# hiroharu-kato/neural_renderer

Measured on AMD Instinct MI355X. Metric: rasterize fwd+bwd Mpixels/sec @256x256 batch=64, higher is better.
Workload: dtype f32

## Files before the change

neural_renderer_amd/csrc/nr_backward_pixel_map.hip:

```cpp
#include "nr_device.h"
#include "nr_band_lines.h"
#include "nr_face_gather.h"
#include "nr_k6_tune.h"

#include <atomic>
#include <mutex>
#include <type_traits>

using namespace nr;

namespace {

constexpr int GRP = 10;
constexpr int NGRP = 6;

struct __attribute__((aligned(16))) LineRec {
    int in_rng;
    int out_rng;
    int base;
    int flags;
    float cross, c0, c1, pad;
    float in_c[4];
    float out_c[4];
};
// ... 350 lines not shown
}

__global__ __launch_bounds__(VIS_CHUNK) void k_compact_visible(const unsigned char *__restrict__ flags,
                                                               const int *__restrict__ chunk_count,
                                                               int *__restrict__ vis_list, int *__restrict__ vis_count,
                                                               int *__restrict__ slot_of, int F, int n_chunks,
                                                               const float *__restrict__ faces,
                                                               unsigned *__restrict__ rng, double *__restrict__ scratch,
                                                               int S, int *__restrict__ band_lines, int n_bands, int W,
                                                               int lds_counters, float *__restrict__ zero_faces,
                                                               int zero_listed)
{
    extern __shared__ int s_band[];
    __shared__ int s_wcnt[VIS_CHUNK / 64];
    __shared__ int s_part[VIS_CHUNK / 64];
    const int b = blockIdx.y, chunk = blockIdx.x, tid = threadIdx.x, lane = tid & 63, wave = tid >> 6;
    if (lds_counters)
        for (int i = tid; i < 2 * n_bands; i += VIS_CHUNK) s_band[i] = 0;
    int part = 0;
    for (int c = tid; c < chunk; c += VIS_CHUNK) part += chunk_count[(size_t)b * n_chunks + c];
#pragma unroll
    for (int o = 32; o > 0; o >>= 1) part += __shfl_xor(part, o, WAVE);
    const int fn = chunk * VIS_CHUNK + tid;
    const bool v = fn < F && flags[(size_t)b * F + fn] != 0;
    const unsigned long long m = __ballot(v);
    if (lane == 0) { s_part[wave] = part; s_wcnt[wave] = __popcll(m); }
    __syncthreads();
    int off = 0, own = 0;
    for (int w = 0; w < VIS_CHUNK / 64; ++w) {
        off += s_part[w];
        if (w < wave) off += s_wcnt[w];
        own += s_wcnt[w];
    }
    if (fn < F) {
        const int before = off + __popcll(m & ((1ull << lane) - 1ull));
        slot_of[(size_t)b * F + fn] = v ? before : -1;
        if (zero_faces && (!v || zero_listed)) zero_face(zero_faces + ((size_t)b * F + fn) * 9);
        if (v)
            emit_visible(b, fn, before, F, S, faces, vis_list, rng, scratch,
                         lds_counters ? s_band : band_lines + (size_t)b * 2 * n_bands, n_bands, W);
    }
    if (lds_counters) {
        __syncthreads();
        for (int i = tid; i < 2 * n_bands; i += VIS_CHUNK) {
            const int c = s_band[i];
            if (c) atomicAdd(band_lines + (size_t)b * 2 * n_bands + i, c);
        }
    }
    if (chunk == n_chunks - 1 && tid == 0) {
        int base = 0;
        for (int w = 0; w < VIS_CHUNK / 64; ++w) base += s_part[w];
        vis_count[b] = base + own;
    }
}

template <int NT>
__device__ __forceinline__ int block_excl_scan(int v, int *s_tmp, int *total)
{
    const int tid = threadIdx.x, lane = tid & 63, wave = tid >> 6;
    int inc = v;
#pragma unroll
    for (int o = 1; o < 64; o <<= 1) {
        const int t = __shfl_up(inc, o, WAVE);
        if (lane >= o) inc += t;
    }
    if (lane == 63) s_tmp[wave] = inc;
    __syncthreads();
    int woff = 0, tot = 0;
    for (int w = 0; w < NT / 64; ++w) {
        const int c = s_tmp[w];
        if (w < wave) woff += c;
        tot += c;
    }
    __syncthreads();
    *total = tot;
    return woff + inc - v;
}

__device__ __forceinline__ double signed_eps(float dist, unsigned eps_hi, unsigned eps_lo)
{
    return __hiloint2double((int)((0.0f < dist) ? eps_hi : (eps_hi ^ 0x80000000u)), (int)eps_lo);
}

__global__ __launch_bounds__(256) void k_line_setup(LineSetupArgs a) { line_setup_body(a, (int)blockIdx.x, (int)blockIdx.y); }

__device__ __forceinline__ void band_prefix(const int *cnt, int n2, int *__restrict__ start_out, int *__restrict__ cursor_out,
                                            int *__restrict__ ok_out, size_t cap)
{
    if (threadIdx.x >= 64) return;
    const int lane = threadIdx.x, per = (n2 + 63) / 64;
    int local = 0;
    for (int i = lane * per; i < min(n2, (lane + 1) * per); ++i) local += cnt[i];
    int inc = local;
#pragma unroll
    for (int o = 1; o < 64; o <<= 1) {
        const int t = __shfl_up(inc, o, WAVE);
        if (lane >= o) inc += t;
    }
    int run = inc - local;
    for (int i = lane * per; i < min(n2, (lane + 1) * per); ++i) {
        start_out[i] = run;
        cursor_out[i] = 0;
        run += cnt[i];
    }
    const int total = __shfl(inc, 63, WAVE);
    if (lane == 0) *ok_out = ((size_t)total <= cap) ? 1 : 0;
}

__global__ __launch_bounds__(256) void k_band_scan(const int *__restrict__ band_lines, int *__restrict__ band_start,
                                                   int *__restrict__ band_cursor, int *__restrict__ lines_ok, int n_bands,
                                                   size_t cap, int force_scan)
{
    const size_t o = (size_t)blockIdx.x * 2 * n_bands;
    band_prefix(band_lines + o, 2 * n_bands, band_start + o, band_cursor + o, lines_ok + blockIdx.x, force_scan ? 0 : cap);
}

__global__ __launch_bounds__(256) void k_band_total(const int *__restrict__ chunk_band, int n_sum, int *__restrict__ band_lines,
                                                    int *__restrict__ band_start, int *__restrict__ lines_ok, int n_bands)
{
    const int b = blockIdx.x, n2 = 2 * n_bands;
    const int *rows = chunk_band + (size_t)b * n_sum * n2;
    for (int i = threadIdx.x; i < n2; i += blockDim.x) {
        int t = 0;
        for (int c = 0; c < n_sum; ++c) t += rows[(size_t)c * n2 + i];
        band_lines[(size_t)b * n2 + i] = t;
        band_start[(size_t)b * n2 + i] = 0;
    }
    if (threadIdx.x == 0) lines_ok[b] = 0;
}

struct FastPx {
    int *fi;
    float *g;
    float *c;
    float *bg;
    unsigned *cov;
    int CW;
    int *span;
};

template <bool RGB, bool ALPHA, int NT>
__device__ __forceinline__ void fast_stage(const FastPx &px, const int32_t *__restrict__ fi_map,
                                           const float *__restrict__ rgb_map, const float *__restrict__ alpha_map,
                                           const float *__restrict__ g_rgb, const float *__restrict__ g_alpha, size_t img,
                                           int axis, int band_lo, int nld, int S, int SP)
{
    const int tid = threadIdx.x;
    auto put = [&](int ld, int d1, int fi, float al, float ga, float r, float g, float bl, float gr, float gg, float gb) {
        const int l = ld * SP + d1;
        px.fi[l] = fi;
        if (RGB) {
            *reinterpret_cast<float4 *>(px.g + 4 * (size_t)l) = make_float4(ga, gr, gg, gb);
            *reinterpret_cast<float4 *>(px.c + 4 * (size_t)l) = make_float4(al, r, g, bl);
            if (px.bg && fi < 0) *reinterpret_cast<float4 *>(px.bg) = make_float4(al, r, g, bl);
        } else {
            px.g[l] = ga;
            px.c[l] = al;
            if (px.bg && fi < 0) px.bg[0] = al;
        }
        if (px.cov && fi >= 0) atomicOr(px.cov + ld * px.CW + (d1 >> 5), 1u << (d1 & 31));
    };
    auto put_quad = [&](size_t g, int ld0, int d10, int ld_step, int d1_step) {
        const int4 vf = *reinterpret_cast<const int4 *>(fi_map + g);
        float4 va = make_float4(0, 0, 0, 0), vg = va;
        if (ALPHA) {
            va = *reinterpret_cast<const float4 *>(alpha_map + g);
            vg = *reinterpret_cast<const float4 *>(g_alpha + g);
// ... 1105 lines not shown
                            __builtin_amdgcn_sched_barrier(0);
                            visit(gC, pC, pf + (float)(2 * SEG), a0, a1);
                            used(gC);
                            visit(gD, pD, pf + (float)(3 * SEG), b0, b1);
                            used(gD);
                            __builtin_amdgcn_sched_barrier(0);
                            gp += 4 * (SEG * NC * 4);
                            pp += 4 * SEG;
                            pf += (float)(4 * SEG);
                        }
                        if (const int rem = steps2 - s) {
                            if (rem == 3) load(2, gC, pC);
                            visit(gA, pA, pf, a0, a1);
                            used(gA);
                            if (rem >= 2) {
                                visit(gB, pB, pf + (float)SEG, b0, b1);
                                used(gB);
                            }
                            if (rem == 3) {
                                visit(gC, pC, pf + (float)(2 * SEG), a0, a1);
                                used(gC);
                            }
                        }
                    }
                    A0 = __builtin_amdgcn_mfma_f64_4x4x4f64((double)a0, 1.0, 0.0, 0, 0, 0);
                    A1 = __builtin_amdgcn_mfma_f64_4x4x4f64((double)a1, 1.0, 0.0, 0, 0, 0);
                    A0 = __builtin_amdgcn_mfma_f64_4x4x4f64((double)b0, 1.0, A0, 0, 0, 0);
                    A1 = __builtin_amdgcn_mfma_f64_4x4x4f64((double)b1, 1.0, A1, 0, 0, 0);
                    A0 = __builtin_amdgcn_mfma_f64_4x4x4f64(A0, 1.0, 0.0, 0, 0, 0);
                    A1 = __builtin_amdgcn_mfma_f64_4x4x4f64(A1, 1.0, 0.0, 0, 0, 0);
                }
                if (act && lane == (row << 2)) acc[src] = make_double2(A0, A1);
            }
            wave_lds_handover();
            if (lane < nw) {
                double2 a = make_double2(0.0, 0.0);
                if (has_b && ((pos >> 2) & (team - 1)) == member) a = acc[lane];
                a.x += (double)f0;
                a.y += (double)f1;
                const bool tneg = !dpos;
                const bool neg0 = EXACT || (((__float_as_uint(qq.y) >> 31) != 0) != tneg);
                const bool neg1 = EXACT || (((__float_as_uint(qq.z) >> 31) != 0) != tneg);
                const double t0 = (flags & 2) ? in0 + (neg0 ? a.x : -a.x) : 0.0;
                const double t1 = (flags & 4) ? in1 + (neg1 ? a.y : -a.y) : 0.0;
                const int tgt = hh.w, lpos = tgt & 0x0fffffff;
                double *dst = scratch + ((size_t)b * F + lpos) * 6 + (1 - axis);
                if (t0 != 0.0) atomicAdd(dst + 2 * ((tgt >> 28) & 3), t0);
                if (t1 != 0.0) atomicAdd(dst + 2 * ((tgt >> 30) & 3), t1);
            }
            wave_lds_handover();
        }
    }
}

template <bool RGB, bool ALPHA, int MODE, bool CHUNKED>
__global__ __launch_bounds__(rowk::NT, MODE == K6_FAST ? 5 : 4) void k_bpm_row(
    const int32_t *__restrict__ fi_map, const float *__restrict__ rgb_map, const float *__restrict__ alpha_map,
    const float *__restrict__ g_rgb, const float *__restrict__ g_alpha, double *__restrict__ scratch,
    const int *__restrict__ band_lines, const int *__restrict__ band_start, const int *__restrict__ lines_ok,
    const BandLine *__restrict__ line_buf, size_t cap, int F, int S, int W, int CH, float eps_f, double eps_d, int B,
    uint4 *__restrict__ zero16, size_t n_zero16)
{
    bpm_row_body<RGB, ALPHA, MODE, CHUNKED, false>(fi_map, rgb_map, alpha_map, g_rgb, g_alpha, scratch, band_lines, band_start, lines_ok,
                                                   line_buf, cap, F, S, W, CH, eps_f, eps_d, B, zero16, n_zero16, nullptr, 1u);
}

struct BandRowArgs {
    const int32_t *fi_map;
    const float *rgb_map, *alpha_map, *g_rgb, *g_alpha;
    double *scratch;
    const int *band_lines, *band_start, *lines_ok;
    const BandLine *line_buf;
    size_t cap;
    int F, S, W, B;
    float eps_f;
    double eps_d;
    uint4 *zero16;
    size_t n_zero16;
    const int *zero_slot;
    unsigned zero_epf;
};

template <bool RGB, bool ALPHA, bool DEPTH>
__global__ __launch_bounds__(rowk::NT, 5) void k_band_gather(BandRowArgs r, FaceGatherArgs g, unsigned band_grid, unsigned gather_x)
{
    if (blockIdx.x < band_grid) {
        bpm_row_body<RGB, ALPHA, K6_FAST, false, true>(r.fi_map, r.rgb_map, r.alpha_map, r.g_rgb, r.g_alpha, r.scratch, r.band_lines,
                                                       r.band_start, r.lines_ok, r.line_buf, r.cap, r.F, r.S, r.W, r.S, r.eps_f, r.eps_d,
                                                       r.B, r.zero16, r.n_zero16, r.zero_slot, r.zero_epf);
    } else {
        const unsigned id = blockIdx.x - band_grid;
        face_gather_body<true, DEPTH, false>(g, (int)(id % gather_x), (int)(id / gather_x));
    }
}

__global__ __launch_bounds__(256) void k_bpm_finalize(const double *__restrict__ scratch, const int *__restrict__ slot_of,
                                                      float *__restrict__ grad_faces, int F, int n_faces_total, int add)
{
    const int i = blockIdx.x * blockDim.x + threadIdx.x;
    if (i >= n_faces_total) return;
    const int pos = slot_of[i];
    float *o = grad_faces + (size_t)i * 9;
    if (add) {
        if (pos < 0) return;
        const double *src = scratch + ((size_t)(i / F) * F + pos) * 6;
#pragma unroll
        for (int v = 0; v < 3; v++) {
            o[3 * v + 0] = (float)src[2 * v + 0] + o[3 * v + 0];
            o[3 * v + 1] = (float)src[2 * v + 1] + o[3 * v + 1];
        }
        return;
    }
    double a[6] = {0.0, 0.0, 0.0, 0.0, 0.0, 0.0};
    if (pos >= 0) {
        const double *src = scratch + ((size_t)(i / F) * F + pos) * 6;
#pragma unroll
        for (int k = 0; k < 6; k++) a[k] = src[k];
    }
#pragma unroll
    for (int v = 0; v < 3; v++) {
        o[3 * v + 0] = (float)a[2 * v + 0];
        o[3 * v + 1] = (float)a[2 * v + 1];
        o[3 * v + 2] = 0.0f;
    }
}


struct BpmLayout {
    size_t flags_off, scratch_off, count_off, chunk_off, cband_off, list_off, rng_off, slot_off, band_off, start_off, cursor_off, ok_off,
        lines_off, total, cap;
    int n_chunks;
};

size_t line_capacity(int F, int S)
{
    const size_t want = (size_t)8 * F + (size_t)32 * S + (size_t)(1.2 * (double)S * sqrt((double)F));
    return (want + 2047 - 1088) / 2048 * 2048 + 1088;
}

BpmLayout bpm_layout(int B, int F, int S)
{
    BpmLayout L;
    const size_t n = (size_t)B * F;
    L.flags_off = 0;
    L.scratch_off = align_up(n, 256);
    L.count_off = align_up(L.scratch_off + n * 6 * sizeof(double), 256);
    L.n_chunks = (F + VIS_CHUNK - 1) / VIS_CHUNK;
    L.chunk_off = L.count_off + align_up((size_t)B * sizeof(int), 256);
    L.cband_off = L.chunk_off + align_up((size_t)B * L.n_chunks * sizeof(int), 256);
    L.list_off = L.cband_off + (L.n_chunks <= SMALL_CHUNKS ? align_up((size_t)B * L.n_chunks * 2 * S * sizeof(int), 256) : 0);
    L.rng_off = L.list_off + align_up(n * sizeof(int), 256);
    L.slot_off = L.rng_off + align_up(n * 6 * sizeof(unsigned), 256);
    const size_t per_band = align_up((size_t)B * 2 * S * sizeof(int), 256);
    L.band_off = L.slot_off + align_up(n * sizeof(int), 256);
    L.start_off = L.band_off + per_band;
    L.cursor_off = L.start_off + per_band;
    L.ok_off = L.cursor_off + per_band;
    L.lines_off = L.ok_off + align_up((size_t)B * sizeof(int), 256);
    L.cap = line_capacity(F, S);
    L.total = L.lines_off + (size_t)B * L.cap * sizeof(BandLine);
    return L;
}

struct ListsLayout {
    size_t count_off, list_off, total;
};
ListsLayout lists_layout(int B, int F)
{
    ListsLayout L;
    L.count_off = 0;
    L.list_off = align_up((size_t)B * sizeof(int), 256);
    L.total = L.list_off + (size_t)B * F * sizeof(int);
    return L;
}

// ... 63 lines not shown
    return (rgb && alpha) ? by_mode(T(), T()) : (rgb ? by_mode(T(), N()) : by_mode(N(), T()));
}

template <bool RGB, bool ALPHA, int MODE, bool OVF>
int launch_fast(const K6Plan &p, const BackwardCall &c, const K6Lists &l, const LineSetupArgs &ls, void *zero_ptr, size_t zero_bytes)
{
    const int B = c.B, S = c.S;
    const unsigned total_wg = (unsigned)((S + p.W_fast - 1) / p.W_fast) * 2u * (unsigned)B;
    const unsigned grid = OVF ? (total_wg < k6::OVF_GRID ? total_wg : k6::OVF_GRID) : xcd_grid(total_wg);
    auto go = [&](auto nt) {
        constexpr int NT = decltype(nt)::value;
        static LdsLimit limit;
        auto kern = k_bpm_fast<RGB, ALPHA, MODE, NT, OVF>;
        if (int rc = limit.ensure((const void *)kern, p.fast_lds)) return rc;
        hipLaunchKernelGGL(kern, dim3(grid), dim3(NT), p.fast_lds, c.st, c.faces, c.face_index_map, c.rgb_map, c.alpha_map,
                           c.grad_rgb_map, c.grad_alpha_map, l.vis_list, l.vis_count, ls.rng, l.scratch, ls.band_lines, ls.band_start,
                           ls.lines_ok, ls.line_buf, ls.cap, c.F, S, p.W_fast, S + 4, c.eps, ls.k2s, B, p.win_lines, p.qcap,
                           (uint4 *)zero_ptr, zero_bytes / 16);
        return 0;
    };
    return p.shape.threads == 256 ? go(std::integral_constant<int, 256>()) : go(std::integral_constant<int, 512>());
}

constexpr int ROW_CHUNK_PX = 512;
int row_chunk(int S, int F)
{
    if (F >= (1 << 15)) return (S + 31) & ~31;
    const int n_ch = (S + ROW_CHUNK_PX - 1) / ROW_CHUNK_PX, len = (S + n_ch - 1) / n_ch;
    return (len + 31) & ~31;
}

int row_band_config(int S, int F, bool rgb, bool exact, int B, size_t *lds_bytes)
{
    if ((((size_t)S + 31) & ~(size_t)31) / rowk::SEG > (size_t)rowk::MAX_SEGS) return 0;
    const size_t SP = (size_t)row_chunk(S, F), n_ch = ((size_t)S + SP - 1) / SP;
    for (int W = rowk::NW; W >= 1; W >>= 1) {
        const size_t wgs = (size_t)B * 2 * ((S + W - 1) / W) * n_ch;
        if ((W > 2 && wgs < k6::ROW_MIN_WGS) || (W == 2 && wgs < k6::ROW_MIN_WGS_1)) continue;
        if ((size_t)W * SP > (size_t)rowk::MAX_PX) continue;
        const size_t npx = (size_t)W * SP;
        *lds_bytes = rgb ? (exact ? rowk::lds_bytes<true, true>(npx) : rowk::lds_bytes<true, false>(npx))
                         : (exact ? rowk::lds_bytes<false, true>(npx) : rowk::lds_bytes<false, false>(npx));
        return W;
    }
    return 0;
}

template <bool RGB, bool ALPHA, int MODE>
int launch_row(const K6Plan &p, const BackwardCall &c, const K6Lists &l, const LineSetupArgs &ls, void *zero_ptr, size_t zero_bytes)
{
    const int B = c.B, F = c.F, S = c.S;
    const double eps = c.eps;
    const int CH = row_chunk(S, F), W = p.W_row;
    const unsigned n_ch = (unsigned)((S + CH - 1) / CH), total_wg = (unsigned)((S + W - 1) / W) * 2u * (unsigned)B * n_ch;
    auto go = [&](auto chunked) {
        constexpr bool C = decltype(chunked)::value;
        static LdsLimit limit;
        if (int rc = limit.ensure((const void *)k_bpm_row<RGB, ALPHA, MODE, C>, p.row_lds)) return rc;
        hipLaunchKernelGGL((k_bpm_row<RGB, ALPHA, MODE, C>), dim3(xcd_grid(total_wg)), dim3(rowk::NT), p.row_lds, c.st,
                           c.face_index_map, c.rgb_map, c.alpha_map, c.grad_rgb_map, c.grad_alpha_map, l.scratch, ls.band_lines,
                           ls.band_start, ls.lines_ok, ls.line_buf, ls.cap, F, S, W, CH, (float)eps, eps, B, (uint4 *)zero_ptr,
                           zero_bytes / 16);
        return 0;
    };
    return n_ch > 1 ? go(std::true_type()) : go(std::false_type());
}

template <bool RGB, bool ALPHA>
int launch_band_gather(const K6Plan &p, const BackwardCall &c, const BackwardPlan &bp, const K6Lists &l, const LineSetupArgs &ls,
                       void *fill, size_t fill_bytes)
{
    const int B = c.B, F = c.F, S = c.S, W = p.W_row;
    const unsigned total_wg = (unsigned)((S + W - 1) / W) * 2u * (unsigned)B, band_grid = xcd_grid(total_wg);
    const unsigned gather_x = (unsigned)((F + 15) / 16);
    const BandRowArgs ra = {c.face_index_map, c.rgb_map, c.alpha_map, c.grad_rgb_map, c.grad_alpha_map, l.scratch, ls.band_lines,
                            ls.band_start, ls.lines_ok, ls.line_buf, ls.cap, F, S, W, B, (float)c.eps, c.eps, (uint4 *)fill,
                            fill_bytes / 16, l.slot_of, 6u};
    const FaceGatherArgs ga = face_gather_args(c, bp, l);
    auto go = [&](auto depth) {
        constexpr bool D = decltype(depth)::value;
        static LdsLimit limit;
        if (int rc = limit.ensure((const void *)k_band_gather<RGB, ALPHA, D>, p.row_lds)) return rc;
        hipLaunchKernelGGL((k_band_gather<RGB, ALPHA, D>), dim3(band_grid + gather_x * (unsigned)B), dim3(rowk::NT), p.row_lds, c.st,
                           ra, ga, band_grid, gather_x);
        return 0;
    };
    return bp.depth_in_gather ? go(std::true_type()) : go(std::false_type());
}

int k6_row_band(int B, int F, int S, bool rgb, double eps, int flags, size_t *row_lds)
{
    const bool exact = (flags & NR_FLAG_EXACT_GRADIENT) != 0;
    const bool possible = !(flags & (NR_FLAG_K6_SCAN | NR_FLAG_K6_LEGACY)) && B <= 65535 && (exact || (float)eps >= 1e-30f);
    return possible ? row_band_config(S, F, rgb, exact, B, row_lds) : 0;
}

}

K6Plan nr::plan_k6(int B, int F, int S, bool rgb, double eps, int flags)
{
    K6Plan p = {};
    const bool exact = (flags & NR_FLAG_EXACT_GRADIENT) != 0;
    p.mode = !exact ? K6_FAST : ((S & (S - 1)) == 0 ? K6_EXACT_POW2 : K6_EXACT);
    p.shape = band_shape(S);
    int w_max = p.shape.w_max, win = BAND_WIN;
    while (w_max > 1 && (size_t)B * 2 * ((S + w_max - 1) / w_max) < 3072) w_max >>= 1;
    p.W_fast = fast_band_config(S, rgb, p.shape, w_max, &p.fast_lds, &win, &p.qcap);
    if (p.W_fast == 0 || (flags & NR_FLAG_K6_GLOBAL)) {
        p.kernel = K6_KERNEL_GLOBAL;
        return p;
    }
    p.win_lines = min(win, max(4, min(BAND_WIN, (int)(65535ll * FSEG / (2ll * S))) & ~3));
    p.W_row = k6_row_band(B, F, S, rgb, eps, flags, &p.row_lds);
    const bool row = p.W_row > 0;
    p.kernel = row ? K6_KERNEL_ROW : K6_KERNEL_FAST;
    p.overflow_pass = row;
    p.row_chunked = row && row_chunk(S, F) < S;
    p.W = row ? 1 : p.W_fast;
    p.n_bands = (S + p.W - 1) / p.W;
    p.use_records = !(flags & NR_FLAG_K6_SCAN) && B <= 65535 && p.n_bands <= 3072;
    const int W_band = row ? p.W_row : p.W_fast;
    const size_t band_wgs = (size_t)((S + W_band - 1) / W_band) * 2 * (size_t)B;
    p.fill_max = band_wgs * ((size_t)k6::FOLD_KB << 10) * (size_t)(row ? rowk::NT : p.shape.threads) / 512;
    return p;
}

NR_API size_t nr_backward_workspace_bytes(int32_t B, int32_t F, int32_t S, int32_t return_rgb, int32_t return_alpha)
{
    if (check_sizes(B, F, S)) return 0;
    if (!return_rgb && !return_alpha) return lists_layout(B, F).total;
    return bpm_layout(B, F, S).total;
}

#ifdef NR_PROFILE_HOOK
#include "../../include/nr_hip_profile.h"
namespace {
struct BandKernelTimer {
    bool on = false, recorded = false;
    int which = -1;
    hipEvent_t start = nullptr, stop = nullptr;
} g_band_timer;
}

NR_API int nr_profile_band_kernel(int32_t enable)
{
    BandKernelTimer &t = g_band_timer;
    if (enable && !t.start) {
        if (hipEventCreate(&t.start) != hipSuccess || hipEventCreate(&t.stop) != hipSuccess) {
            t.start = t.stop = nullptr;
            return launch_status();
        }
    }
    t.on = enable != 0 && t.start != nullptr;
    t.recorded = false;
    return 0;
}

NR_API float nr_profile_band_kernel_ms(void)
{
    BandKernelTimer &t = g_band_timer;
    float ms = -1.0f;
    if (!t.recorded || hipEventSynchronize(t.stop) != hipSuccess || hipEventElapsedTime(&ms, t.start, t.stop) != hipSuccess) {
        (void)hipGetLastError();
        return -1.0f;
    }
    return ms;
}
// ... 2 lines not shown
{
    (void)return_alpha;
    return plan_k6(B, F, S, return_rgb != 0, eps, flags).kernel == K6_KERNEL_ROW ? 1 : 0;
}
#define NR_BAND_TIMER_START(st, kernel) if (g_band_timer.on) { g_band_timer.which = (kernel); g_band_timer.recorded = hipEventRecord(g_band_timer.start, st) == hipSuccess; }
#define NR_BAND_TIMER_STOP(st) if (g_band_timer.on && g_band_timer.recorded) g_band_timer.recorded = hipEventRecord(g_band_timer.stop, st) == hipSuccess
#else
#define NR_BAND_TIMER_START(st, kernel) ((void)0)
#define NR_BAND_TIMER_STOP(st) ((void)0)
#endif


static bool compact_in_one_launch(const BpmLayout &L, int n_bands) { return L.n_chunks <= SMALL_CHUNKS && n_bands <= 4096; }

int nr::k6_compact(const BackwardCall &c, const K6Plan &plan, int face_zeros, K6Lists &out)
{
    const int B = c.B, F = c.F, S = c.S, n = B * F;
    const BpmLayout L = bpm_layout(B, F, S);
    const hipStream_t st = c.st;
    unsigned char *ws = (unsigned char *)c.workspace;
    int *band_lines = (int *)(ws + L.band_off);
    const int W = plan.W, n_bands = plan.n_bands;
    double *scratch = (double *)(ws + L.scratch_off);
    int *vis_count = (int *)(ws + L.count_off);
    int *vis_list = (int *)(ws + L.list_off);
    int *slot_of = (int *)(ws + L.slot_off);
    unsigned *rng = (unsigned *)(ws + L.rng_off);
    out = {vis_list, vis_count, slot_of, scratch};
    const unsigned char *vflags = c.visible_faces;
    if (!vflags) {
        unsigned char *f = ws + L.flags_off;
        const int he = fill_bytes(f, 0, (size_t)n, st);
        if (he != 0) return he;
        const size_t P = (size_t)B * S * S;
        hipLaunchKernelGGL(k_mark_visible, dim3((unsigned)((P + 255) / 256)), dim3(256), 0, st, c.face_index_map, f, F,
                           S * S, P);
        vflags = f;
    }
    int *band_start = (int *)(ws + L.start_off), *band_cursor = (int *)(ws + L.cursor_off), *lines_ok = (int *)(ws + L.ok_off);
    float *zero_faces = face_zeros != FACE_ZEROS_NONE ? c.grad_faces : nullptr;
    const int zero_listed = face_zeros == FACE_ZEROS_ALL ? 1 : 0;
    if (compact_in_one_launch(L, n_bands)) {
        int *chunk_band = (int *)(ws + L.cband_off);
        const int use_diff = (size_t)(2 * n_bands + 2 * (S + 1)) * sizeof(int) <= 40960 ? 1 : 0;
        hipLaunchKernelGGL(k_compact_par, dim3((unsigned)L.n_chunks, (unsigned)B), dim3(VIS_CHUNK),
                           (size_t)(2 * n_bands + (use_diff ? 2 * (S + 1) : 0)) * sizeof(int), st, vflags, vis_list, vis_count,
                           slot_of, F, L.n_chunks, c.faces, rng, scratch, S, chunk_band, n_bands, W, band_cursor, zero_faces,
                           zero_listed, use_diff);
        if (!plan.use_records)
            hipLaunchKernelGGL(k_band_total, dim3((unsigned)B), dim3(256), 0, st, chunk_band, L.n_chunks, band_lines, band_start,
                               lines_ok, n_bands);
    } else {
        int *chunk_count = (int *)(ws + L.chunk_off);
        hipLaunchKernelGGL(k_count_visible, dim3((unsigned)L.n_chunks, (unsigned)B), dim3(VIS_CHUNK), 0, st, vflags,
                           chunk_count, F, L.n_chunks, band_lines, n_bands);
        const int lds_counters = n_bands <= 4096;
        hipLaunchKernelGGL(k_compact_visible, dim3((unsigned)L.n_chunks, (unsigned)B), dim3(VIS_CHUNK),
                           lds_counters ? (size_t)2 * n_bands * sizeof(int) : 0, st, vflags, chunk_count, vis_list, vis_count,
                           slot_of, F, L.n_chunks, c.faces, rng, scratch, S, band_lines, n_bands, W, lds_counters, zero_faces,
                           zero_listed);
        hipLaunchKernelGGL(k_band_scan, dim3((unsigned)B), dim3(256), 0, st, band_lines, band_start, band_cursor, lines_ok,
                           n_bands, plan.use_records ? L.cap : 0, 0);
    }
    return launch_status();
}

LineSetupArgs nr::k6_line_setup_args(const BackwardCall &c, const K6Plan &plan)
{
    const BpmLayout L = bpm_layout(c.B, c.F, c.S);
    unsigned char *ws = (unsigned char *)c.workspace;
    const int n_bands = plan.n_bands;
    const float k2s = (c.flags & NR_FLAG_EXACT_GRADIENT) ? 1.0f : 2.0f / (float)c.S;
    return {c.faces, c.face_index_map, (const int *)(ws + L.list_off), (const int *)(ws + L.count_off),
            (const unsigned *)(ws + L.rng_off), (const int *)(ws + L.cband_off), compact_in_one_launch(L, n_bands) ? L.n_chunks : 0,
            (int *)(ws + L.band_off), (int *)(ws + L.start_off), (int *)(ws + L.cursor_off), (int *)(ws + L.ok_off),
            (BandLine *)(ws + L.lines_off), L.cap, c.F, c.S, plan.W, n_bands, k2s, (unsigned)((c.F + LS_FACES - 1) / LS_FACES),
            (unsigned)c.B, (size_t)6 * n_bands * sizeof(int)};
}

int nr::run_line_setup(const LineSetupArgs &a, hipStream_t st)
{
    static LdsLimit ls_limit;
    if (int rc = ls_limit.ensure((const void *)k_line_setup, a.lds_bytes)) return rc;
    hipLaunchKernelGGL(k_line_setup, dim3(a.grid_x, a.grid_y), dim3(256), a.lds_bytes, st, a);
    return launch_status();
}

int nr::k6_band(const BackwardCall &c, const K6Plan &plan, const K6Lists &l, const LineSetupArgs &ls, void *fill, size_t fill_bytes,
                const BackwardPlan *tail)
{
    if (plan.kernel == K6_KERNEL_GLOBAL) {
        auto global = [&](auto r, auto a) {
            hipLaunchKernelGGL((k_bpm_global<decltype(r)::value, decltype(a)::value>), dim3((unsigned)(c.B * c.F)), dim3(WAVE), 0,
                               c.st, c.faces, c.face_index_map, c.rgb_map, c.alpha_map, c.grad_rgb_map, c.grad_alpha_map,
                               c.grad_faces, c.F, c.S, c.eps);
            return launch_status();
        };
        using T = std::true_type;
        using N = std::false_type;
        return (c.rgb && c.alpha) ? global(T(), T()) : (c.rgb ? global(T(), N()) : global(N(), T()));
    }
    auto band_fast = [&](auto overflow_only, void *zp, size_t zb) {
        return with_k6_types(c.rgb, c.alpha, plan.mode, [&](auto r, auto a, auto m) {
            return launch_fast<decltype(r)::value, decltype(a)::value, decltype(m)::value, decltype(overflow_only)::value>(
                plan, c, l, ls, zp, zb);
        });
    };
    auto band_row = [&]() {
        return with_k6_types(c.rgb, c.alpha, plan.mode, [&](auto r, auto a, auto m) {
            return launch_row<decltype(r)::value, decltype(a)::value, decltype(m)::value>(plan, c, l, ls, fill, fill_bytes);
        });
    };
    auto band_gather = [&]() {
        auto go = [&](auto r, auto a) {
            return launch_band_gather<decltype(r)::value, decltype(a)::value>(plan, c, *tail, l, ls, fill, fill_bytes);
        };
        using T = std::true_type;
        using N = std::false_type;
        return (c.rgb && c.alpha) ? go(T(), T()) : (c.rgb ? go(T(), N()) : go(N(), T()));
    };
    NR_BAND_TIMER_START(c.st, plan.kernel);
    int rc = tail ? band_gather() : (plan.kernel == K6_KERNEL_ROW ? band_row() : band_fast(std::false_type(), fill, fill_bytes));
    NR_BAND_TIMER_STOP(c.st);
    if (rc == 0 && plan.overflow_pass) rc = band_fast(std::true_type(), nullptr, 0);
    return rc ? rc : launch_status();
}

void nr::k6_finalize(const BackwardCall &c, const K6Lists &l, bool add)
{
    const int n = c.B * c.F;
    hipLaunchKernelGGL(k_bpm_finalize, dim3((unsigned)((n + 255) / 256)), dim3(256), 0, c.st, l.scratch, l.slot_of, c.grad_faces,
                       c.F, n, add ? 1 : 0);
}

bool nr::k6_lists_fit(int B, int F, size_t workspace_bytes)
{
    return workspace_bytes >= lists_layout(B, F).total && (F + VIS_CHUNK - 1) / VIS_CHUNK <= SMALL_CHUNKS;
}

K6Lists nr::k6_list_visible(const BackwardCall &c)
{
    const ListsLayout L = lists_layout(c.B, c.F);
    const int n_chunks = (c.F + VIS_CHUNK - 1) / VIS_CHUNK;
    unsigned char *ws = (unsigned char *)c.workspace;
    int *list = (int *)(ws + L.list_off), *count = (int *)(ws + L.count_off);
    hipLaunchKernelGGL(k_list_visible, dim3((unsigned)n_chunks, (unsigned)c.B), dim3(VIS_CHUNK), 0, c.st, c.visible_faces, list,
                       count, c.F, n_chunks);
    return {list, count, nullptr, nullptr};
}
```

neural_renderer_amd/csrc/nr_band_lines.h:

```cpp
#pragma once
#include "nr_device.h"

namespace nr {

struct __attribute__((aligned(16))) BandLine {
    int in_rng;
    int out_rng;
    int geo;
    int tgt;
    float cross, c0, c1;
    int fn;
};

struct LineSetupArgs {
    const float *faces;
    const int32_t *fi_map;
    const int *vis_list, *vis_count;
    const unsigned *rng;
    const int *chunk_band;
    int n_sum;
    int *band_lines, *band_start, *band_cursor, *lines_ok;
    BandLine *line_buf;
    size_t cap;
    int F, S, W, n_bands;
    float k2s;
    unsigned grid_x, grid_y;
    size_t lds_bytes;
};

namespace {


constexpr unsigned RNG_EMPTY = 1u;

__device__ __forceinline__ unsigned edge_range(float p0x, float p1x, int S)
{
    const int d0_from = (int)fmax((double)ceilf(fminf(p0x, p1x)), 0.0);
    const int d0_to = (int)fmin((double)fmaxf(p0x, p1x), S - 1.0);
    return (p0x != p1x && d0_to >= d0_from) ? (unsigned)d0_from | ((unsigned)d0_to << 16) : RNG_EMPTY;
}


struct LineHead {
    float p0x, p0y, p1x, p1y, p2x, p2y, d0f, d1_cross;
    int direction, d1_in, d1_out;
    bool live;
};

__device__ __forceinline__ LineHead fast_line_head(const float *__restrict__ fv, int e, int axis, int d0, int S)
{
    const float fs = (float)S;
    const int i0 = e, i1 = (e + 1) % 3, i2 = (e + 2) % 3;
    float fp[6];
#pragma unroll
    for (int k = 0; k < 3; k++) { fp[k] = to_pixel(fv[3 * k], fs); fp[3 + k] = to_pixel(fv[3 * k + 1], fs); }
    const int ox = axis ? 3 : 0, oy = axis ? 0 : 3;
    LineHead h;
    h.p0x = fp[ox + i0]; h.p0y = fp[oy + i0]; h.p1x = fp[ox + i1]; h.p1y = fp[oy + i1];
    h.p2x = fp[ox + i2]; h.p2y = fp[oy + i2];
    if (axis == 0) h.direction = (h.p0x < h.p1x) ? -1 : 1; else h.direction = (h.p0x < h.p1x) ? 1 : -1;
    h.d0f = (float)d0;
    h.d1_cross = (h.p1y - h.p0y) / (h.p1x - h.p0x) * (h.d0f - h.p0x) + h.p0y;
    h.d1_in = (0 < h.direction) ? (int)floorf(h.d1_cross) : (int)ceilf(h.d1_cross);
    h.d1_out = h.d1_in + h.direction;
    h.live = !(h.d1_in < 0 || S <= h.d1_in) && !(h.d1_out < 0 || S <= h.d1_out);
    return h;
}

__device__ __forceinline__ BandLine fast_line_finish(const LineHead &h, int ld, int S, int rfn, int tgt, int owner, float k2s)
{
    const float p0x = h.p0x, p0y = h.p0y, p1x = h.p1x, p1y = h.p1y, p2x = h.p2x, p2y = h.p2y, d0f = h.d0f;
    const int direction = h.direction, d1_in = h.d1_in, d1_out = h.d1_out;
    BandLine r;
    r.in_rng = 1; r.out_rng = 1; r.geo = 0; r.tgt = tgt;
    r.cross = r.c0 = r.c1 = 0.0f;
    r.fn = rfn;
    if (h.live) {
        int flags = (0 < direction) ? 8 : 0;
        if (p1x != d0f) flags |= 2;
        if (p0x != d0f) flags |= 4;
        r.c0 = (p1x - p0x) / (p1x - d0f) * k2s;
        r.c1 = (p1x - p0x) / (d0f - p0x) * k2s;
        if (owner == rfn) {
            const int lim = (0 < direction) ? S - 1 : 0;
            const int o_from = max(min(d1_out, lim), 0), o_to = min(max(d1_out, lim), S - 1);
            r.out_rng = o_from | (o_to << 16);
            flags |= 1;
        }
        float d0_cross2;
        if ((d0f - p0x) * (d0f - p2x) < 0)
            d0_cross2 = (p2y - p0y) / (p2x - p0x) * (d0f - p0x) + p0y;
        else
            d0_cross2 = (p1y - p2y) / (p1x - p2x) * (d0f - p2x) + p2y;
        const int lim2 = (0 < direction) ? (int)ceilf(d0_cross2) : (int)floorf(d0_cross2);
        const int i_from = max(min(d1_in, lim2), 0), i_to = min(max(d1_in, lim2), S - 1);
        r.in_rng = i_from | (i_to << 16);
        r.geo = d1_in | (ld << 16) | (flags << 24);
        r.cross = h.d1_cross;
    }
    return r;
}

template <typename OwnerOf>
__device__ __forceinline__ BandLine make_fast_line(const float *__restrict__ fv, int e, int axis, int d0, int ld, int S,
                                                   int rfn, int tgt, OwnerOf owner_of, float k2s)
{
    const LineHead h = fast_line_head(fv, e, axis, d0, S);
    return fast_line_finish(h, ld, S, rfn, tgt, h.live ? owner_of(h.d1_in) : -1, k2s);
}

constexpr int LS_UNROLL = 4;
constexpr int LS_FACES = 32;

__device__ __forceinline__ int band_sum_prefix(const int *__restrict__ rows, int n_sum, int n2, int *tot, int *start,
                                               int *s_tmp)
{
    const int tid = threadIdx.x, lane = tid & 63, wave = tid >> 6;
    for (int i = tid; i < n2; i += 256) {
        int t = 0;
        for (int c = 0; c < n_sum; ++c) t += rows[(size_t)c * n2 + i];
        tot[i] = t;
    }
    __syncthreads();
    const int per = (n2 + 255) / 256, i0 = tid * per, i1 = min(n2, i0 + per);
    int local = 0;
    for (int i = i0; i < i1; ++i) local += tot[i];
    int inc = local;
#pragma unroll
    for (int o = 1; o < 64; o <<= 1) {
        const int t = __shfl_up(inc, o, WAVE);
        if (lane >= o) inc += t;
    }
    if (lane == 63) s_tmp[wave] = inc;
    __syncthreads();
    int run = inc - local;
    for (int w = 0; w < wave; ++w) run += s_tmp[w];
    for (int i = i0; i < i1; ++i) {
        start[i] = run;
        run += tot[i];
    }
    const int total = s_tmp[0] + s_tmp[1] + s_tmp[2] + s_tmp[3];
    __syncthreads();
    return total;
}

__device__ __forceinline__ void line_setup_body(const LineSetupArgs &a, const int bx, const int by)
{
    const float *__restrict__ faces = a.faces;
    const int32_t *__restrict__ fi_map = a.fi_map;
    const int *__restrict__ vis_list = a.vis_list, *__restrict__ vis_count = a.vis_count;
    const unsigned *__restrict__ rng = a.rng;
    const int *__restrict__ chunk_band = a.chunk_band;
    const int n_sum = a.n_sum;
    int *__restrict__ band_lines = a.band_lines, *__restrict__ band_start = a.band_start, *__restrict__ band_cursor = a.band_cursor,
        *__restrict__ lines_ok = a.lines_ok;
    BandLine *__restrict__ line_buf = a.line_buf;
    const size_t cap = a.cap;
    const int F = a.F, S = a.S, W = a.W, n_bands = a.n_bands;
    const float k2s = a.k2s;
    extern __shared__ int s_cnt[];
    int *s_base = s_cnt + 2 * n_bands;
    int *s_start = s_base + 2 * n_bands;
    __shared__ int s_tmp[4];
    __shared__ unsigned s_rng[6 * LS_FACES];
    __shared__ int s_lp[6 * LS_FACES + 1];
    __shared__ int s_fn[LS_FACES];
    __shared__ float s_face[9 * LS_FACES];
    const int b = by, tid = threadIdx.x;
    const bool first = bx == 0;
    const int n_vis = vis_count[b];
    const int n_wg = (n_vis + LS_FACES - 1) / LS_FACES;
    const int pos0 = bx, pstep = n_wg;
    const int n_pos = bx < n_wg ? (n_vis - pos0 + pstep - 1) / pstep : 0;
    if (n_pos == 0 && !first) return;
    unsigned r_own = RNG_EMPTY;
    int fn_own = 0;
    if (tid < 6 * n_pos) {
        const int p = tid / 6, ae = tid - 6 * p, axis = ae / 3, e = ae - 3 * axis;
        r_own = rng[(((size_t)b * 2 + axis) * F + pos0 + p * pstep) * 3 + e];
    }
    if (tid < n_pos) fn_own = vis_list[(size_t)b * F + pos0 + tid * pstep];
    int ok;
    if (n_sum > 0) {
        const int total = band_sum_prefix(chunk_band + (size_t)b * n_sum * 2 * n_bands, n_sum, 2 * n_bands, s_cnt, s_start, s_tmp);
        ok = (size_t)total <= cap ? 1 : 0;
        if (first) {
            for (int i = tid; i < 2 * n_bands; i += 256) {
                band_lines[(size_t)b * 2 * n_bands + i] = s_cnt[i];
                band_start[(size_t)b * 2 * n_bands + i] = s_start[i];
            }
            if (tid == 0) lines_ok[b] = ok;
        }
    } else {
        ok = lines_ok[b];
        for (int i = tid; i < 2 * n_bands; i += 256) s_start[i] = band_start[(size_t)b * 2 * n_bands + i];
    }
    if (n_pos == 0 || !ok) return;
    __syncthreads();
    for (int i = tid; i < 2 * n_bands; i += 256) s_cnt[i] = 0;
    if (tid < 6 * LS_FACES) s_rng[tid] = r_own;
    if (tid < LS_FACES) s_fn[tid] = fn_own;
    __syncthreads();
    float fv_a = 0.0f, fv_b = 0.0f;
    {
        const int p = tid / 9, k = tid - 9 * p;
        if (p < n_pos) fv_a = faces[((size_t)b * F + s_fn[p]) * 9 + k];
        const int t2 = tid + 256, p2 = t2 / 9, k2 = t2 - 9 * p2;
        if (t2 < 9 * LS_FACES && p2 < n_pos) fv_b = faces[((size_t)b * F + s_fn[p2]) * 9 + k2];
    }
    {
        int lines = 0;
        if (tid < 6 * n_pos) {
            const int p = tid / 6, ae = tid - 6 * p, axis = ae / 3;
            const unsigned pr = s_rng[tid];
            const int lo = (int)(pr & 0xffffu), hi = (int)(pr >> 16);
            for (int band = lo / W; band * W <= hi; ++band)
                atomicAdd(s_cnt + axis * n_bands + band, min(hi, band * W + W - 1) - max(lo, band * W) + 1);
            lines = hi >= lo ? hi - lo + 1 : 0;
        }
        const int lane = tid & 63, wave = tid >> 6;
        int inc = lines;
#pragma unroll
        for (int o = 1; o < 64; o <<= 1) {
            const int t = __shfl_up(inc, o, WAVE);
            if (lane >= o) inc += t;
        }
        if (lane == 63) s_tmp[wave] = inc;
        __syncthreads();
        int before = 0;
        for (int w = 0; w < wave; ++w) before += s_tmp[w];
        if (tid < 6 * LS_FACES) s_lp[tid] = before + inc - lines;
        if (tid == 6 * LS_FACES - 1) s_lp[6 * LS_FACES] = before + inc;
    }
    __syncthreads();
    for (int i = tid; i < 2 * n_bands; i += 256) {
        const int c = s_cnt[i];
        s_base[i] = c > 0 ? s_start[i] + atomicAdd(band_cursor + (size_t)b * 2 * n_bands + i, c) : 0;
        s_cnt[i] = 0;
    }
    s_face[tid] = fv_a;
    if (tid + 256 < 9 * LS_FACES) s_face[tid + 256] = fv_b;
    __syncthreads();
    const size_t img = (size_t)b * S * S;
    BandLine *buf_b = line_buf + (size_t)b * cap;
    const int n_items = 6 * n_pos, n_lines = s_lp[n_items];
    for (int base = 0; base < n_lines; base += LS_UNROLL * 256) {
        LineHead h[LS_UNROLL];
        int item[LS_UNROLL], d0v[LS_UNROLL], own[LS_UNROLL];
#pragma unroll
        for (int u = 0; u < LS_UNROLL; u++) {
            const int l = base + u * 256 + tid;
            item[u] = -1;
            own[u] = -1;
            if (l < n_lines) {
                int lo = 0, hi = n_items;
                while (hi - lo > 1) {
                    const int mid = (lo + hi) >> 1;
                    if (s_lp[mid] <= l) lo = mid; else hi = mid;
                }
                item[u] = lo;
                const int p = lo / 6, ae = lo - 6 * p, axis = ae / 3, e = ae - 3 * axis;
                const int d0 = (int)(s_rng[lo] & 0xffffu) + (l - s_lp[lo]);
                d0v[u] = d0;
                float fv[9];
#pragma unroll
                for (int k = 0; k < 9; k++) fv[k] = s_face[9 * p + k];
                h[u] = fast_line_head(fv, e, axis, d0, S);
                if (h[u].live) own[u] = fi_map[axis ? img + (size_t)d0 * S + h[u].d1_in : img + (size_t)h[u].d1_in * S + d0];
            }
        }
#pragma unroll
        for (int u = 0; u < LS_UNROLL; u++) {
            if (item[u] < 0) continue;
            const int p = item[u] / 6, ae = item[u] - 6 * p, axis = ae / 3, e = ae - 3 * axis;
            const int band = d0v[u] / W, ld = d0v[u] - band * W;
            const int tgt = (pos0 + p * pstep) | (e << 28) | (((e + 1) % 3) << 30);
            const int bi = axis * n_bands + band;
            buf_b[s_base[bi] + atomicAdd(s_cnt + bi, 1)] = fast_line_finish(h[u], ld, S, s_fn[p], tgt, own[u], k2s);
        }
    }
}

}
}
```

neural_renderer_amd/csrc/nr_device.h:

```cpp
#pragma once
#include <hip/hip_runtime.h>
#include <stdint.h>
#include <stdlib.h>

#include "../../include/nr_hip.h"

#define NR_API extern "C" __attribute__((visibility("default")))

namespace nr {

constexpr int WAVE = 64;


__device__ __forceinline__ bool is_backside(float x0, float y0, float x1, float y1, float x2, float y2)
{
    return (y2 - y0) * (x1 - x0) < (y1 - y0) * (x2 - x0);
}

__device__ __forceinline__ float to_pixel(float v, float fs) { return 0.5f * (v * fs + fs - 1.0f); }

__device__ __forceinline__ void compute_face_inv(const float px[3], const float py[3], float inv[9])
{
    inv[0] = py[1] - py[2];
    inv[1] = px[2] - px[1];
// ... 211 lines not shown
    const int32_t *face_image = nullptr;
    const float *base = nullptr;
    int ts = 0, M = 0, P = 0;
    int shared = 0;
};

struct UVSample {
    int m, f0;
    int q[4];
    float w[4];
    Taps t;
};

__device__ __forceinline__ void corner_weights(const float (&z)[3], const float (&w)[3], float zp, float (&d)[3])
{
#pragma unroll
    for (int k = 0; k < 3; k++) d[k] = fminf(fmaxf(w[k] * (zp / z[k]), 0.0f), 1.0f);
}

__device__ __forceinline__ void uv_locate(const UVShade &uv, int fi, int tex_faces, const float *face, float w0, float w1,
                                          float w2, float zp, double eps, UVSample &s)
{
    const bool flip = fi >= tex_faces;
    s.f0 = flip ? fi - tex_faces : fi;
    const int m = uv.face_image[s.f0];
    s.m = (m >= 0 && m < uv.M) ? m : -1;
    const float fz[3] = {face[2], face[5], face[8]};
    const float w[3] = {w0, w1, w2};
    if (s.m < 0) {
        compute_taps(fz, w, zp, uv.ts, eps, s.t, flip);
        return;
    }
    float d[3];
#pragma unroll
    for (int k = 0; k < 3; k++) d[k] = fminf(fmaxf(w[k] * (zp / fz[k]), 0.0f), 1.0f);
    if (flip) {
        const float d0 = d[0];
        d[0] = d[2];
        d[2] = d0;
    }
    const int off = uv.table[3 * s.m], H = uv.table[3 * s.m + 1], W = uv.table[3 * s.m + 2];
    long long p[4];
    texel_reads(uv.faces_uv + (size_t)s.f0 * 6, d, H, W, p, s.w);
#pragma unroll
    for (int r = 0; r < 4; r++) s.q[r] = off + mirror_row(p[r], H, W);
}

__device__ __forceinline__ void uv_color(const UVShade &uv, const UVSample &s, int b, float c[3])
{
    c[0] = c[1] = c[2] = 0.0f;
    if (s.m >= 0) {
        const float *img = uv.images + (uv.shared ? 0 : (size_t)b * uv.P * 3);
#pragma unroll
        for (int r = 0; r < 4; r++) {
            const float *px = img + (size_t)s.q[r] * 3;
            c[0] += px[0] * s.w[r];
            c[1] += px[1] * s.w[r];
            c[2] += px[2] * s.w[r];
        }
        return;
    }
    const int T = uv.ts * uv.ts * uv.ts;
    const float *texture = uv.base + (size_t)s.f0 * T * 3;
#pragma unroll
    for (int pn = 0; pn < 8; pn++) {
        if (s.t.isc[pn] >= T) continue;
        const float *tx = texture + s.t.isc[pn] * 3;
        c[0] += s.t.w[pn] * tx[0];
        c[1] += s.t.w[pn] * tx[1];
        c[2] += s.t.w[pn] * tx[2];
    }
}


constexpr unsigned NUM_XCD = 8;
inline unsigned xcd_grid(size_t n_blocks) { return (unsigned)((n_blocks + NUM_XCD - 1) / NUM_XCD * NUM_XCD); }
#ifdef __HIPCC__
__device__ __forceinline__ unsigned xcd_block(unsigned n_blocks)
{
    const unsigned chunk = (n_blocks + NUM_XCD - 1) / NUM_XCD;
    const unsigned logical = (blockIdx.x % NUM_XCD) * chunk + blockIdx.x / NUM_XCD;
    return logical < n_blocks ? logical : n_blocks;
}
#endif

inline size_t align_up(size_t v, size_t a) { return (v + a - 1) / a * a; }

#ifdef __HIPCC__
static __global__ __launch_bounds__(256) void k_fill_bytes(unsigned char *__restrict__ dst, size_t bytes, unsigned value32)
{
    const size_t i0 = ((size_t)blockIdx.x * blockDim.x + threadIdx.x) * 16;
    if (i0 >= bytes) return;
    if (i0 + 16 <= bytes && ((size_t)(dst + i0) & 15) == 0) {
        *reinterpret_cast<uint4 *>(dst + i0) = make_uint4(value32, value32, value32, value32);
    } else {
        for (size_t i = i0; i < bytes && i < i0 + 16; ++i) dst[i] = (unsigned char)value32;
    }
}
inline int fill_bytes(void *dst, int byte, size_t bytes, hipStream_t st)
{
    if (bytes == 0) return 0;
    const unsigned b = (unsigned)(byte & 0xff), v = b | (b << 8) | (b << 16) | (b << 24);
    hipLaunchKernelGGL(k_fill_bytes, dim3((unsigned)((bytes + 4095) / 4096)), dim3(256), 0, st, (unsigned char *)dst, bytes, v);
    return (int)hipGetLastError();
}
#endif

inline int check_sizes(int B, int F, int S)
{
    if (B < 1 || B > 65535 || F < 1 || S < 1 || S > 16384) return NR_E_SIZE;
    if ((size_t)B * (size_t)F > 0x7fffffffull / 9) return NR_E_SIZE;
    return 0;
}

inline int launch_status()
{
    const hipError_t e = hipGetLastError();
    return e == hipSuccess ? 0 : (int)e;
}


enum { STAGE_K6 = 1, STAGE_K7 = 2, STAGE_K8 = 4, STAGE_ALL = 7 };

struct BackwardCall {
    int stages;
    bool rgb, alpha;
    const float *faces, *faces_z_ref;
    const int32_t *face_index_map;
    const float *weight_map, *depth_map, *rgb_map, *alpha_map, *grad_rgb_map, *grad_alpha_map, *grad_depth_map;
    const float *sampling_weight_map;
    const int32_t *sampling_index_map;
    const float *face_inv_map;
    float *grad_faces, *grad_textures;
    int B, F, S, ts;
    double eps;
    int flags;
    const unsigned char *visible_faces;
    void *workspace;
    size_t workspace_bytes;
    FaceLight lit;
    hipStream_t st;
};

struct BandShape {
    int threads;
    int w_max;
    size_t budget;
};
enum K6Kernel { K6_KERNEL_FAST = 0, K6_KERNEL_ROW = 1, K6_KERNEL_GLOBAL = 2 };
struct K6Plan {
    int kernel;
    int mode;
    BandShape shape;
    int W_fast;
    size_t fast_lds;
    int win_lines, qcap;
    int W_row;
    size_t row_lds;
    int W, n_bands;
    bool use_records;
    bool overflow_pass;
    bool row_chunked;
    size_t fill_max;
};
K6Plan plan_k6(int B, int F, int S, bool rgb, double eps, int flags);

// ... 57 lines not shown
```

Measured before the change: 15210.

## Shrink line-setup register state, reorder block-to-image mapping, raise occupancy hint

The line-setup kernel stops holding a full LineHead per unrolled slot across the atomic phase. It keeps only the packed item/d0, the crossing value and d1_in, then recomputes the endpoint pixels in the second pass, and its launch bounds now request 8 blocks per CU. Both line setup and the face-gather part of the band kernel now map linear block ids so the image index varies fastest, meant to spread each face chunk across images and XCDs. The change trades a little recomputation for lower register pressure and higher occupancy. The different block order may change cache locality.

```diff
diff --git a/neural_renderer_amd/csrc/nr_backward_pixel_map.hip b/neural_renderer_amd/csrc/nr_backward_pixel_map.hip
--- a/neural_renderer_amd/csrc/nr_backward_pixel_map.hip
+++ b/neural_renderer_amd/csrc/nr_backward_pixel_map.hip
@@ -456,7 +456,11 @@
     return __hiloint2double((int)((0.0f < dist) ? eps_hi : (eps_hi ^ 0x80000000u)), (int)eps_lo);
 }
 
-__global__ __launch_bounds__(256) void k_line_setup(LineSetupArgs a) { line_setup_body(a, (int)blockIdx.x, (int)blockIdx.y); }
+__global__ __launch_bounds__(256, 8) void k_line_setup(LineSetupArgs a)
+{
+    const SlotImage w = image_fastest(blockIdx.x, a.grid_y);
+    line_setup_body(a, w.bx, w.by);
+}
 
 __device__ __forceinline__ void band_prefix(const int *cnt, int n2, int *__restrict__ start_out, int *__restrict__ cursor_out,
                                             int *__restrict__ ok_out, size_t cap)
@@ -1728,15 +1732,15 @@
 };
 
 template <bool RGB, bool ALPHA, bool DEPTH>
-__global__ __launch_bounds__(rowk::NT, 5) void k_band_gather(BandRowArgs r, FaceGatherArgs g, unsigned band_grid, unsigned gather_x)
+__global__ __launch_bounds__(rowk::NT, 5) void k_band_gather(BandRowArgs r, FaceGatherArgs g, unsigned band_grid)
 {
     if (blockIdx.x < band_grid) {
         bpm_row_body<RGB, ALPHA, K6_FAST, false, true>(r.fi_map, r.rgb_map, r.alpha_map, r.g_rgb, r.g_alpha, r.scratch, r.band_lines,
                                                        r.band_start, r.lines_ok, r.line_buf, r.cap, r.F, r.S, r.W, r.S, r.eps_f, r.eps_d,
                                                        r.B, r.zero16, r.n_zero16, r.zero_slot, r.zero_epf);
     } else {
-        const unsigned id = blockIdx.x - band_grid;
-        face_gather_body<true, DEPTH, false>(g, (int)(id % gather_x), (int)(id / gather_x));
+        const SlotImage w = image_fastest(blockIdx.x - band_grid, (unsigned)r.B);
+        face_gather_body<true, DEPTH, false>(g, w.bx, w.by);
     }
 }
 
@@ -1966,7 +1970,7 @@
         static LdsLimit limit;
         if (int rc = limit.ensure((const void *)k_band_gather<RGB, ALPHA, D>, p.row_lds)) return rc;
         hipLaunchKernelGGL((k_band_gather<RGB, ALPHA, D>), dim3(band_grid + gather_x * (unsigned)B), dim3(rowk::NT), p.row_lds, c.st,
-                           ra, ga, band_grid, gather_x);
+                           ra, ga, band_grid);
         return 0;
     };
     return bp.depth_in_gather ? go(std::true_type()) : go(std::false_type());
@@ -2135,7 +2139,7 @@
 {
     static LdsLimit ls_limit;
     if (int rc = ls_limit.ensure((const void *)k_line_setup, a.lds_bytes)) return rc;
-    hipLaunchKernelGGL(k_line_setup, dim3(a.grid_x, a.grid_y), dim3(256), a.lds_bytes, st, a);
+    hipLaunchKernelGGL(k_line_setup, dim3(a.grid_x * a.grid_y), dim3(256), a.lds_bytes, st, a);
     return launch_status();
 }
 
diff --git a/neural_renderer_amd/csrc/nr_band_lines.h b/neural_renderer_amd/csrc/nr_band_lines.h
--- a/neural_renderer_amd/csrc/nr_band_lines.h
+++ b/neural_renderer_amd/csrc/nr_band_lines.h
@@ -47,7 +47,7 @@
     bool live;
 };
 
-__device__ __forceinline__ LineHead fast_line_head(const float *__restrict__ fv, int e, int axis, int d0, int S)
+__device__ __forceinline__ void line_head_points(LineHead &h, const float *__restrict__ fv, int e, int axis, int d0, int S)
 {
     const float fs = (float)S;
     const int i0 = e, i1 = (e + 1) % 3, i2 = (e + 2) % 3;
@@ -55,11 +55,16 @@
 #pragma unroll
     for (int k = 0; k < 3; k++) { fp[k] = to_pixel(fv[3 * k], fs); fp[3 + k] = to_pixel(fv[3 * k + 1], fs); }
     const int ox = axis ? 3 : 0, oy = axis ? 0 : 3;
-    LineHead h;
     h.p0x = fp[ox + i0]; h.p0y = fp[oy + i0]; h.p1x = fp[ox + i1]; h.p1y = fp[oy + i1];
     h.p2x = fp[ox + i2]; h.p2y = fp[oy + i2];
     if (axis == 0) h.direction = (h.p0x < h.p1x) ? -1 : 1; else h.direction = (h.p0x < h.p1x) ? 1 : -1;
     h.d0f = (float)d0;
+}
+
+__device__ __forceinline__ LineHead fast_line_head(const float *__restrict__ fv, int e, int axis, int d0, int S)
+{
+    LineHead h;
+    line_head_points(h, fv, e, axis, d0, S);
     h.d1_cross = (h.p1y - h.p0y) / (h.p1x - h.p0x) * (h.d0f - h.p0x) + h.p0y;
     h.d1_in = (0 < h.direction) ? (int)floorf(h.d1_cross) : (int)ceilf(h.d1_cross);
     h.d1_out = h.d1_in + h.direction;
@@ -111,6 +116,7 @@
 
 constexpr int LS_UNROLL = 4;
 constexpr int LS_FACES = 32;
+static_assert(9 * LS_FACES >= 256, "line_setup_body stores s_face[tid] for every thread of the workgroup");
 
 __device__ __forceinline__ int band_sum_prefix(const int *__restrict__ rows, int n_sum, int n2, int *tot, int *start,
                                                int *s_tmp)
@@ -244,42 +250,59 @@
     const size_t img = (size_t)b * S * S;
     BandLine *buf_b = line_buf + (size_t)b * cap;
     const int n_items = 6 * n_pos, n_lines = s_lp[n_items];
+    static_assert(6 * LS_FACES <= 256, "item | d0 << 8");
     for (int base = 0; base < n_lines; base += LS_UNROLL * 256) {
-        LineHead h[LS_UNROLL];
-        int item[LS_UNROLL], d0v[LS_UNROLL], own[LS_UNROLL];
+        float cross[LS_UNROLL];
+        int item_d0[LS_UNROLL], d1_in[LS_UNROLL], own[LS_UNROLL];
 #pragma unroll
         for (int u = 0; u < LS_UNROLL; u++) {
             const int l = base + u * 256 + tid;
-            item[u] = -1;
+            item_d0[u] = -1;
             own[u] = -1;
+            d1_in[u] = -1;
+            cross[u] = 0.0f;
             if (l < n_lines) {
                 int lo = 0, hi = n_items;
                 while (hi - lo > 1) {
                     const int mid = (lo + hi) >> 1;
                     if (s_lp[mid] <= l) lo = mid; else hi = mid;
                 }
-                item[u] = lo;
                 const int p = lo / 6, ae = lo - 6 * p, axis = ae / 3, e = ae - 3 * axis;
                 const int d0 = (int)(s_rng[lo] & 0xffffu) + (l - s_lp[lo]);
-                d0v[u] = d0;
+                item_d0[u] = lo | (d0 << 8);
                 float fv[9];
 #pragma unroll
                 for (int k = 0; k < 9; k++) fv[k] = s_face[9 * p + k];
-                h[u] = fast_line_head(fv, e, axis, d0, S);
-                if (h[u].live) own[u] = fi_map[axis ? img + (size_t)d0 * S + h[u].d1_in : img + (size_t)h[u].d1_in * S + d0];
+                const LineHead h = fast_line_head(fv, e, axis, d0, S);
+                cross[u] = h.d1_cross;
+                if (h.live) {
+                    d1_in[u] = h.d1_in;
+                    own[u] = fi_map[axis ? img + (size_t)d0 * S + h.d1_in : img + (size_t)h.d1_in * S + d0];
+                }
             }
         }
+        asm volatile("" ::: "memory");
 #pragma unroll
         for (int u = 0; u < LS_UNROLL; u++) {
-            if (item[u] < 0) continue;
-            const int p = item[u] / 6, ae = item[u] - 6 * p, axis = ae / 3, e = ae - 3 * axis;
-            const int band = d0v[u] / W, ld = d0v[u] - band * W;
+            if (item_d0[u] < 0) continue;
+            const int it = item_d0[u] & 255, d0 = item_d0[u] >> 8;
+            const int p = it / 6, ae = it - 6 * p, axis = ae / 3, e = ae - 3 * axis;
+            const int band = d0 / W, ld = d0 - band * W;
             const int tgt = (pos0 + p * pstep) | (e << 28) | (((e + 1) % 3) << 30);
             const int bi = axis * n_bands + band;
-            buf_b[s_base[bi] + atomicAdd(s_cnt + bi, 1)] = fast_line_finish(h[u], ld, S, s_fn[p], tgt, own[u], k2s);
-        }
-    }
-}
-
-}
-}
+            float fv[9];
+#pragma unroll
+            for (int k = 0; k < 9; k++) fv[k] = s_face[9 * p + k];
+            LineHead h;
+            line_head_points(h, fv, e, axis, d0, S);
+            h.d1_cross = cross[u];
+            h.live = d1_in[u] >= 0;
+            h.d1_in = d1_in[u];
+            h.d1_out = h.d1_in + h.direction;
+            buf_b[s_base[bi] + atomicAdd(s_cnt + bi, 1)] = fast_line_finish(h, ld, S, s_fn[p], tgt, own[u], k2s);
+        }
+    }
+}
+
+}
+}
diff --git a/neural_renderer_amd/csrc/nr_device.h b/neural_renderer_amd/csrc/nr_device.h
--- a/neural_renderer_amd/csrc/nr_device.h
+++ b/neural_renderer_amd/csrc/nr_device.h
@@ -317,6 +317,13 @@
     const unsigned logical = (blockIdx.x % NUM_XCD) * chunk + blockIdx.x / NUM_XCD;
     return logical < n_blocks ? logical : n_blocks;
 }
+
+struct SlotImage { int bx, by; };
+__device__ __forceinline__ SlotImage image_fastest(unsigned id, unsigned B)
+{
+    const unsigned bx = id / B;
+    return {(int)bx, (int)(id - bx * B)};
+}
 #endif
 
 inline size_t align_up(size_t v, size_t a) { return (v + a - 1) / a * a; }
```

New measurement: 16100 (median of 6 runs). 1.06x the previous value.
